# stelleg/caster-dta

Measured on AMD Instinct MI355X. Metric: graph-pairs/sec (Davis-shaped protein+drug), encoders fwd+bwd, higher is better.
Workload: dtype f32; 1 GPU; davis_b64; pairs_per_gpu=64, residues_per_gpu=19200, protein_edges_per_gpu=57484, atoms_per_gpu=2560, drug_edges_per_gpu=7986, encoder=CASTER-DTA(2,2), pass=fwdbwd, activation_storage=fp32, scope=encoders, torch_compile=False, tunable_gemms=False, two_lane_head=False, train_mode=True, csr_build_in_step=True, hip_graph=True, kernels=mfma

## Files before the change

caster-dta_amd/csrc/gvp_internal.h:

```cpp
#pragma once
#include <hip/hip_runtime.h>
#include <stdint.h>

#include "gvp_host.h"
#include "gvp_math.h"
#include "gvp_rng.h"

constexpr int POLICY_F32 = 0, POLICY_BF16 = 1, POLICY_GVPDEF = 2, POLICY_LINEAR = 3;

struct QuadOffsets {
  int emb, conv0, node0, layer_stride, head, total;
  int embT, convT0, nodeT0, layerT_stride, headT;
};

#ifndef CGVP_BWD_MAX_GRID
#define CGVP_BWD_MAX_GRID 240
#endif
constexpr int kBwdMaxGrid = CGVP_BWD_MAX_GRID;

#include <type_traits>

namespace gq { struct bf16s; struct f32_gvpdef; struct f32_linear; }
template <class T> struct Tag { using type = T; };
template <class ST> constexpr bool is_layer_kind = std::is_same_v<ST, gq::f32_gvpdef> || std::is_same_v<ST, gq::f32_linear>;
// ... 10 lines not shown
template <class F>
int with_flag(bool b, F&& f) { return b ? f(std::true_type{}) : f(std::false_type{}); }

namespace quad {
int offsets(int nt_node, int nt_edge, int num_convs, QuadOffsets* o);
int prepare(const gvp::EncLayout& L, int num_convs, int packed_bf16, const float* params, float* image, hipStream_t st);
int node_embed(int nt_node, const float* img, const float* x_s, const float* x_v, const int64_t* ntypes,
               int64_t N, float* h, unsigned long long* rng_state, unsigned long long* rng_out, int policy, hipStream_t st);
int pass_begin(const gvp::EncLayout& L, int num_convs, int policy, const float* params, float* image, const float* x_s,
               const float* x_v, const int64_t* ntypes, int64_t N, float* h, unsigned long long* rng_state,
               unsigned long long* rng_out, const int64_t* edge_index, int64_t E, int32_t* counters, hipStream_t st);
int conv(int nt_edge, const float* img, const float* h, const float* e_s, const float* e_v,
         const int64_t* etypes, const int32_t* rowptr, const int32_t* eperm, const int32_t* esrc,
         const int32_t* edst, int64_t N, int64_t E, int mean, float* dh, int fuse, const float* img_node,
         const float* img_head, float* h_out, float* out, const float* mask0, const float* mask1, gvp::RngArgs rng,
         const float* e_in, float* e_out, int policy, hipStream_t st);
int node_update(const float* img_node, const float* img_head, const float* h, const float* dh, int64_t N,
                int with_head, float* h_out, float* out, const float* mask0, const float* mask1, gvp::RngArgs rng,
                int policy, hipStream_t st);

int node_update_bwd(const float* img_node, const float* imgT_node, const float* h, const float* dh,
                    const float* mask0, const float* mask1, gvp::RngArgs rng, const float* g_up0, const float* g_up1,
                    const float* g_up2, int64_t N, float* g_dh, float* g_h, float* zero_rows, float* slab, int* grid,
                    int policy, hipStream_t st);
int head_bwd(const float* img_head, const float* imgT_head, const float* h_out, const float* g_out, int64_t N,
             float* g_h_out, float* slab, int* grid, int policy, hipStream_t st);
int node_head_bwd(const float* img_head, const float* imgT_head, const float* h_out, const float* g_out, float* g_h_out,
                  float* head_slab, const float* img_node, const float* imgT_node, const float* h, const float* dh,
                  const float* mask0, const float* mask1, gvp::RngArgs rng, int64_t N, float* g_dh, float* g_h,
                  float* zero_rows, float* slab, int* grid, int policy, hipStream_t st);
int conv_bwd(int nt_edge, const float* img, const float* imgT, const float* h, const float* e_emb,
// ... 29 lines not shown
             int* row_len, hipStream_t st, const float* agg_in = nullptr, const uint16_t* pos_in = nullptr,
             float* g_edge = nullptr, float* g_self = nullptr,
             float* g_eattr = nullptr, int eattr_accum = 0);
int gine_fwd(int cin, int chid, int cout, int nt, int net, int ed, const float* x, const int64_t* ntypes,
             const float* eattr, const int64_t* etypes, const int32_t* rowptr, const int32_t* eperm,
             const int32_t* esrc, const int32_t* edst, int64_t N, const cgvp_gine_w* w, float slope,
             const float* mask, gvp::RngArgs rng, float* out, float* agg_out, uint16_t* pos_out, hipStream_t st);
int reduce_slab(const float* slab, int rows, int stride, int col0, int len, float* dst, hipStream_t st);
int reduce_segments(const cgvp_segment* segs, int nsegs, float* grad_params, hipStream_t st, int overwrite = 0,
                    bool store_only = false);
struct BwdBlocks { int emb, conv_edge, conv_total, node, head; };
int bwd_block_sizes(int nt_node, int nt_edge, BwdBlocks* b);
void zero_words(void* p, size_t words, hipStream_t s);
int csr_build(const int64_t* edge_index, int64_t N, int64_t E, int32_t* rowptr, int32_t* eperm, int32_t* esrc,
              int32_t* edst, int32_t* work, int work_is_zero, int32_t* ids_scratch, unsigned long long* rng_state,
              unsigned long long* rng_out, hipStream_t stream);
}
```

caster-dta_amd/csrc/gvp_kernels.hip:

```cpp
#include <hip/hip_runtime.h>
#include <stdlib.h>
#include <stdint.h>

#include "gvp_internal.h"

using namespace gvp;

namespace {

constexpr int WAVE = 64;

inline int check_dims(const cgvp_dims* d) {
  if (!d) return CGVP_ERR_BAD_ARG;
  if (d->node_in_s != NODE_IN_S || d->node_in_v != NODE_IN_V || d->edge_in_s != EDGE_IN_S ||
      d->edge_in_v != EDGE_IN_V || d->hidden_s != NS || d->hidden_v != NV ||
      d->edge_hidden_s != ES || d->edge_hidden_v != EV || d->out_s != OUT)
    return CGVP_ERR_UNSUPPORTED_DIMS;
  if (d->storage != CGVP_F32 && d->storage != CGVP_BF16) return CGVP_ERR_UNSUPPORTED_DIMS;
  if (d->layer_kind < CGVP_LAYER_GATED || d->layer_kind > CGVP_LAYER_LINEAR) return CGVP_ERR_UNSUPPORTED_DIMS;
  if (d->layer_kind != CGVP_LAYER_GATED && d->storage != CGVP_F32) return CGVP_ERR_UNSUPPORTED_DIMS;
  return 0;
}
inline int check_dims_gated(const cgvp_dims* d) {
  if (int rc = check_dims(d)) return rc;
// ... 41 lines not shown
  int64_t e = (int64_t)blockIdx.x * blockDim.x + threadIdx.x;
  if (rng_state && e == 0) {
    const unsigned long long off = rng_state[1] + 1;
    rng_state[1] = off;
    rng_out[0] = rng_state[0];
    rng_out[1] = off;
  }
  if (e >= E) return;
  int64_t s = ei[e], d = ei[E + e];
  if (s < 0 || s >= N || d < 0 || d >= N) return;
  atomicAdd(&cnt[d], 1);
}

constexpr int SCAN_LDS = 36 * 1024;
__global__ __launch_bounds__(1024) void csr_scan_kernel(const int32_t* __restrict__ cnt, int64_t N,
                                                        int32_t* __restrict__ rowptr) {
  extern __shared__ int32_t sbuf[];
  const int t = threadIdx.x;
  const int tile_cap = (int)(N < SCAN_LDS ? (N + 3) / 4 * 4 : SCAN_LDS);
  int32_t* part = sbuf + tile_cap;
  int32_t carry = 0;
  for (int64_t base = 0; base < N || base == 0; base += SCAN_LDS) {
    const int64_t rem = N - base;
    const int n = (int)(rem < SCAN_LDS ? (rem > 0 ? rem : 0) : SCAN_LDS);
    constexpr int VPT = SCAN_LDS / 4096;
    int4 v[VPT];
    const int n4 = n >> 2;
    const int4* src4 = reinterpret_cast<const int4*>(cnt + base);
#pragma unroll
    for (int k = 0; k < VPT; ++k) {
      const int q = t + 1024 * k;
      v[k] = q < n4 ? src4[q] : make_int4(0, 0, 0, 0);
    }
// ... 37 lines not shown
        reinterpret_cast<int4*>(rowptr + base)[q] = x;
      }
      if (t < (n & 3)) rowptr[base + (n4 << 2) + t] = sbuf[(n4 << 2) + t];
    } else {
      for (int i = t; i < n; i += 1024) rowptr[base + i] = sbuf[i];
    }
    carry += total;
    __syncthreads();
    if (N == 0) break;
  }
  if (t == 0) rowptr[N] = carry;
}

constexpr int SCAN_MULTI_MAX = 65536, SCAN_MULTI_T = 256, SCAN_MULTI_CHUNK = 4 * SCAN_MULTI_T;
__global__ __launch_bounds__(SCAN_MULTI_T) void csr_scan_multi_kernel(const int32_t* __restrict__ cnt, int32_t N,
                                                                      int32_t counters, int32_t* __restrict__ rowptr) {
  __shared__ int32_t part[2 * (SCAN_MULTI_T / WAVE)];
  const int t = threadIdx.x, wv = t >> 6;
  const int4* c4 = reinterpret_cast<const int4*>(cnt);
  int32_t pre = 0;
  for (int q = t; q < (int)blockIdx.x * SCAN_MULTI_T; q += SCAN_MULTI_T) {
    const int4 v = c4[q];
    pre += (v.x + v.y) + (v.z + v.w);
  }
  const int i0 = (int)blockIdx.x * SCAN_MULTI_CHUNK + 4 * t;
  const int4 v = i0 < counters ? c4[i0 >> 2] : make_int4(0, 0, 0, 0);
  const int32_t sum = (v.x + v.y) + (v.z + v.w);
  int32_t inc = sum;
#pragma unroll
  for (int off = 1; off < WAVE; off <<= 1) {
    const int32_t u = __shfl_up(inc, off);
    if ((t & (WAVE - 1)) >= off) inc += u;
    pre += __shfl_xor(pre, off);
// ... 14 lines not shown
  }
}

__global__ void csr_fill_kernel(const int64_t* __restrict__ ei, int64_t N, int64_t E, const int32_t* __restrict__ rowptr,
                                int32_t* __restrict__ cnt, int32_t* __restrict__ tmp, int32_t* __restrict__ edst) {
  int64_t e = (int64_t)blockIdx.x * blockDim.x + threadIdx.x;
  if (e >= E) return;
  int64_t s = ei[e], d = ei[E + e];
  if (s < 0 || s >= N || d < 0 || d >= N) return;
  int32_t pos = rowptr[d] + atomicSub(&cnt[d], 1) - 1;
  if (pos < 0 || pos >= E) return;
  tmp[pos] = (int32_t)e;
  edst[pos] = (int32_t)d;
}

__global__ void csr_rank_kernel(const int64_t* __restrict__ ei, int64_t N, int64_t E, int64_t counters,
                                const int32_t* __restrict__ rowptr, const int32_t* __restrict__ tmp,
                                int32_t* __restrict__ edst, int32_t* __restrict__ eperm,
                                int32_t* __restrict__ esrc, int32_t* __restrict__ cnt) {
  const int64_t t = (int64_t)blockIdx.x * blockDim.x + threadIdx.x;
  if (t < counters) cnt[t] = 0;
  if (t >= rowptr[N] || t >= E) {
    if (t < E) { eperm[t] = -1; esrc[t] = 0; edst[t] = 0; }
    return;
  }
  const int32_t n = edst[t];
  if (n < 0 || n >= N) return;
  int32_t lo = rowptr[n], hi = rowptr[n + 1];
  const int32_t key = tmp[t];
  if (lo < 0 || hi > E || lo > hi || key < 0 || key >= E) return;
  int32_t rank = 0;
  for (int32_t j = lo; j < hi; ++j) rank += tmp[j] < key ? 1 : 0;
  eperm[lo + rank] = key;
  esrc[lo + rank] = (int32_t)ei[key];
}

__global__ void src_count_kernel(const int32_t* __restrict__ esrc, const int32_t* __restrict__ rowptr, int64_t N,
                                 int32_t* __restrict__ cnt) {
  const int64_t p = (int64_t)blockIdx.x * blockDim.x + threadIdx.x;
  if (p >= rowptr[N]) return;
  const int32_t s = esrc[p];
  if (s >= 0 && s < N) atomicAdd(&cnt[s], 1);
}
__global__ void src_fill_kernel(const int32_t* __restrict__ esrc, const int32_t* __restrict__ rowptr, int64_t N,
                                const int32_t* __restrict__ sptr, int32_t* __restrict__ cnt, int32_t* __restrict__ tmp) {
  const int64_t p = (int64_t)blockIdx.x * blockDim.x + threadIdx.x;
  const int32_t ev = rowptr[N];
  if (p >= ev) return;
  const int32_t s = esrc[p];
// ... 396 lines not shown
const char* cgvp_build_info(void) { return "libcaster_gvp gfx950 (HIP, wave64), built " __DATE__ " " __TIME__; }

int cgvp_csr_from_coo(const int64_t* edge_index, int64_t N, int64_t E, int32_t* rowptr,
                      int32_t* eperm, int32_t* esrc, int32_t* edst, int32_t* work, int32_t work_is_zero,
                      int32_t* ids_scratch, void* stream) {
  return quad::csr_build(edge_index, N, E, rowptr, eperm, esrc, edst, work, work_is_zero, ids_scratch, nullptr, nullptr,
                         (hipStream_t)stream);
}
}

namespace quad {
void zero_words(void* p, size_t words, hipStream_t s) { ::zero_words(p, words, s); }

int csr_build(const int64_t* edge_index, int64_t N, int64_t E, int32_t* rowptr, int32_t* eperm, int32_t* esrc,
              int32_t* edst, int32_t* work, int work_is_zero, int32_t* ids_scratch, unsigned long long* rng_state,
              unsigned long long* rng_out, hipStream_t stream) {
  if (N < 0 || E < 0 || !rowptr || !work || (E > 0 && (!edge_index || !eperm || !esrc || !edst || !ids_scratch)))
    return CGVP_ERR_BAD_ARG;
  if (N >= (int64_t)1 << 31 || E >= (int64_t)1 << 31) return CGVP_ERR_BAD_ARG;
  if ((uintptr_t)work & 15) return CGVP_ERR_BAD_ARG;
  hipStream_t s = stream;
  const int64_t counters = (N + 1 + 63) / 64 * 64;
  if (work_is_zero == 0) {
    zero_words(work, (size_t)counters, s);
  }
  int32_t* tmp = ids_scratch;
  const int B = 256;
  if (E > 0 && work_is_zero != 2)
    launch<csr_count_kernel>(dim3((unsigned)((E + B - 1) / B)), dim3(B), 0, s, edge_index, N, E, work, rng_state, rng_out);
  else if (rng_state)
    launch<rng_next_kernel>(dim3(1), dim3(1), 0, s, rng_state, rng_out);
  if (N < SCAN_MULTI_MAX) {
    launch<csr_scan_multi_kernel>(dim3((unsigned)((N + 1 + SCAN_MULTI_CHUNK - 1) / SCAN_MULTI_CHUNK)),
                                  dim3(SCAN_MULTI_T), 0, s, work, (int32_t)N, (int32_t)counters, rowptr);
  } else {
    const int64_t tile = N < SCAN_LDS ? (N + 3) / 4 * 4 : SCAN_LDS;
    if (int rc = launch<csr_scan_kernel>(dim3(1), dim3(1024), (size_t)(tile + 1024 + 32) * sizeof(int32_t), s, work, N, rowptr)) return rc;
  }
  if (E > 0) launch<csr_fill_kernel>(dim3((unsigned)((E + B - 1) / B)), dim3(B), 0, s, edge_index, N, E, rowptr, work, tmp, edst);
  const int64_t span = E > counters ? E : counters;
  launch<csr_rank_kernel>(dim3((unsigned)((span + B - 1) / B)), dim3(B), 0, s, edge_index, N, E, counters, rowptr, tmp,
                          edst, eperm, esrc, work);
  return launch_status();
}

bool deterministic_env() {
  static const bool v = [] { const char* e = getenv("CGVP_DETERMINISTIC"); return e && e[0] == '1'; }();
  return v;
}

int64_t src_index_work_ints(int64_t N, int64_t E) { return (N + 1 + 63) / 64 * 64 + (E > 0 ? E : 1); }

int src_index(const int32_t* rowptr, const int32_t* esrc, int64_t N, int64_t E, int32_t* sptr, int32_t* spos,
              int32_t* work, hipStream_t s) {
  if (N < 0 || E < 0 || !rowptr || !sptr || !work || (E > 0 && (!esrc || !spos))) return CGVP_ERR_BAD_ARG;
  if (N >= (int64_t)1 << 31 || E >= (int64_t)1 << 31 || ((uintptr_t)work & 15)) return CGVP_ERR_BAD_ARG;
  const int64_t counters = (N + 1 + 63) / 64 * 64;
  int32_t* cnt = work;
  int32_t* tmp = work + counters;
  zero_words(cnt, (size_t)counters, s);
  const int B = 256;
  const unsigned eb = (unsigned)((E + B - 1) / B);
  if (E > 0) launch<src_count_kernel>(dim3(eb), dim3(B), 0, s, esrc, rowptr, N, cnt);
  if (N < SCAN_MULTI_MAX) {
    launch<csr_scan_multi_kernel>(dim3((unsigned)((N + 1 + SCAN_MULTI_CHUNK - 1) / SCAN_MULTI_CHUNK)),
                                  dim3(SCAN_MULTI_T), 0, s, cnt, (int32_t)N, (int32_t)counters, sptr);
  } else {
    const int64_t tile = N < SCAN_LDS ? (N + 3) / 4 * 4 : SCAN_LDS;
    if (int rc = launch<csr_scan_kernel>(dim3(1), dim3(1024), (size_t)(tile + 1024 + 32) * sizeof(int32_t), s, cnt, N, sptr)) return rc;
  }
  if (E > 0) {
    launch<src_fill_kernel>(dim3(eb), dim3(B), 0, s, esrc, rowptr, N, sptr, cnt, tmp);
    launch<src_rank_kernel>(dim3(eb), dim3(B), 0, s, esrc, rowptr, N, sptr, tmp, spos);
  }
  return launch_status();
}
}

extern "C" {

int cgvp_deterministic_forced(void) { return quad::deterministic_env() ? 1 : 0; }

int cgvp_csr_collate(const int32_t* st_rowptr, const int32_t* st_eperm, const int32_t* st_esrc,
                     const int32_t* st_edst, const int64_t* st_node_off, const int64_t* st_edge_off,
// ... 121 lines not shown
  hipStream_t st = (hipStream_t)stream;
  switch (layout->nt_edge) {
    case 0: launch<conv_fwd_kernel<0>>(grid, dim3(WAVE), 0, st, a); break;
    case 1: launch<conv_fwd_kernel<1>>(grid, dim3(WAVE), 0, st, a); break;
    default: return CGVP_ERR_UNSUPPORTED_DIMS;
  }
  return launch_status();
}

int cgvp_conv_layer_fwd(const cgvp_dims* dims, const cgvp_layout* layout, const float* image, int32_t layer,
                        const float* h, const float* e_s, const float* e_v, const int64_t* etypes,
                        const int32_t* rowptr, const int32_t* eperm, const int32_t* esrc, const int32_t* edst,
                        int64_t N, int64_t E, int32_t aggr_mean, const float* mask0, const float* mask1,
                        const cgvp_rng* rng, int32_t with_head, const float* e_in, float* e_out, float* dh,
                        float* h_out, float* out, void* stream) {
  if (int rc = check_dims_gated(dims)) return rc;
  if (int rc = check_rng(rng)) return rc;
  if (N < 0 || E < 0 || !layout || !image) return CGVP_ERR_BAD_ARG;
  if (layer < 0 || layer >= num_convs_of(*layout)) return CGVP_ERR_BAD_ARG;
  if (N == 0) return 0;
  if (!h || !rowptr || (with_head ? !out : !h_out)) return CGVP_ERR_BAD_ARG;
  if (E > 0 && (!esrc || !edst)) return CGVP_ERR_BAD_ARG;
  if (E > 0 && !e_in && (!e_s || !e_v || !eperm || (layout->nt_edge > 0 && !etypes))) return CGVP_ERR_BAD_ARG;
  const void* al[] = {h, e_s, dh, h_out, out, mask0, mask1, e_in, e_out};
  for (const void* q : al) if ((uintptr_t)q & 15) return CGVP_ERR_BAD_ARG;
  QuadOffsets o;
  if (int rc = quad::offsets(layout->nt_node, layout->nt_edge, num_convs_of(*layout), &o)) return rc;
  if (int rc = quad::conv(layout->nt_edge, image + o.conv0 + layer * o.layer_stride, h, e_s, e_v, etypes, rowptr, eperm,
                          esrc, edst, N, E, aggr_mean ? 1 : 0, dh, with_head ? 2 : 1,
                          image + o.node0 + layer * o.layer_stride, image + o.head, h_out, out, mask0, mask1,
                          rng_args(rng, 2 * layer), e_in, e_in ? nullptr : e_out, policy_of(dims), (hipStream_t)stream)) return rc;
  return launch_status();
}

int cgvp_node_update_fwd(const cgvp_dims* dims, const cgvp_layout* layout, const float* params,
                         const float* image, int32_t layer, const float* h, const float* dh, int64_t N,
                         int32_t with_head, float* h_out, float* out, void* stream) {
  if (int rc = check_dims(dims)) return rc;
  if (N < 0 || !layout || !params) return CGVP_ERR_BAD_ARG;
  if (layer < 0 || layer >= num_convs_of(*layout)) return CGVP_ERR_BAD_ARG;
  if (N == 0) return 0;
  if (!h || !dh || (with_head ? !out : !h_out)) return CGVP_ERR_BAD_ARG;
  if (((uintptr_t)h & 15) || ((uintptr_t)dh & 15)) return CGVP_ERR_BAD_ARG;
  if (image) {
    if (((uintptr_t)h_out & 15) || ((uintptr_t)out & 15)) return CGVP_ERR_BAD_ARG;
    QuadOffsets o;
    if (int rc = quad::offsets(layout->nt_node, layout->nt_edge, num_convs_of(*layout), &o)) return rc;
    if (int rc = quad::node_update(image + o.node0 + layer * o.layer_stride, image + o.head, h, dh, N,
// ... 291 lines not shown
```

caster-dta_amd/csrc/gvp_quad_kernels.hip:

```cpp
#include <hip/hip_runtime.h>
#include <stdlib.h>
#include <stdint.h>

#include "gvp_internal.h"
#include "gvp_quad.h"

using namespace gq;

namespace {

#ifdef CGVP_STAMPS
__device__ unsigned long long* g_stamp_buf = nullptr;
#define STAMP(slot)                                                                          \
  do {                                                                                       \
    __builtin_amdgcn_sched_barrier(0);                                                       \
    unsigned long long t_;                                                                   \
    asm volatile("s_waitcnt vmcnt(0) lgkmcnt(0)\n\ts_memtime %0\n\ts_waitcnt lgkmcnt(0)" : "=s"(t_)::"memory"); \
    __builtin_amdgcn_sched_barrier(0);                                                       \
    if (g_stamp_buf && (threadIdx.x & 63) == 0)                                              \
      g_stamp_buf[((size_t)blockIdx.x * WPB + (threadIdx.x >> 6)) * 16 + (slot)] = t_;        \
  } while (0)
#define STAMP_REAL(slot)                                                                     \
  do {                                                                                       \
    unsigned long long t_;                                                                   \
// ... 20 lines not shown
  f4* d = reinterpret_cast<f4*>(lds);
  f4 v[IT];
#pragma unroll
  for (int k = 0; k < IT; ++k) {
    const int idx = tid + k * TPB;
    if (idx < NF4) v[k] = s[idx];
  }
#pragma unroll
  for (int k = 0; k < IT; ++k) {
    const int idx = tid + k * TPB;
    if (idx < NF4) d[idx] = v[k];
  }
}

template <int N0, int N1, int N2, int TPB = gq_fwd_tpb>
__device__ __forceinline__ void stage_slices(float* lds, const float* __restrict__ s0, const float* __restrict__ s1,
                                             const float* __restrict__ s2, int tid) {
  static_assert(N0 % 4 == 0 && N1 % 4 == 0 && N2 % 4 == 0, "image slices are whole float4s");
  constexpr int F0 = N0 / 4, F1 = N1 / 4, F2 = N2 / 4;
  constexpr int I0 = (F0 + TPB - 1) / TPB, I1 = (F1 + TPB - 1) / TPB, I2 = (F2 + TPB - 1) / TPB;
  f4* d = reinterpret_cast<f4*>(lds);
  f4 v0[I0 > 0 ? I0 : 1], v1[I1 > 0 ? I1 : 1], v2[I2 > 0 ? I2 : 1];
#pragma unroll
  for (int k = 0; k < I0; ++k) { const int idx = tid + k * TPB; if (idx < F0) v0[k] = reinterpret_cast<const f4*>(s0)[idx]; }
#pragma unroll
  for (int k = 0; k < I1; ++k) { const int idx = tid + k * TPB; if (idx < F1) v1[k] = reinterpret_cast<const f4*>(s1)[idx]; }
#pragma unroll
  for (int k = 0; k < I2; ++k) { const int idx = tid + k * TPB; if (idx < F2) v2[k] = reinterpret_cast<const f4*>(s2)[idx]; }
#pragma unroll
  for (int k = 0; k < I0; ++k) { const int idx = tid + k * TPB; if (idx < F0) d[idx] = v0[k]; }
#pragma unroll
  for (int k = 0; k < I1; ++k) { const int idx = tid + k * TPB; if (idx < F1) d[F0 + idx] = v1[k]; }
#pragma unroll
  for (int k = 0; k < I2; ++k) { const int idx = tid + k * TPB; if (idx < F2) d[F0 + F1 + idx] = v2[k]; }
}

template <int NTN, int NTE>
__device__ __forceinline__ float image_element(const float* __restrict__ P, const EncLayout& L, int num_convs, int packed, int idx) {
  typedef Image<NTN, NTE> IM;

  float v;
  if (idx < IM::EMB_SIZE) {
    v = idx < IM::EMB_LN ? QNode<NTN>::element(P + L.node_gvp, idx, packed != 0) : P[L.node_ln + (idx - IM::EMB_LN)];
  } else if (idx < IM::head(num_convs)) {
    const int j = idx - IM::EMB_SIZE;
    const int l = j / (IM::CV_SIZE + IM::ND_SIZE);
    int k = j - l * (IM::CV_SIZE + IM::ND_SIZE);
    const float* C = P + L.conv0 + l * L.conv_stride;
    if (k < IM::CV_SIZE) {
// ... 239 lines not shown
  f4 s[1], m1s;
  float v[3][1], m1v;
  node_inputs<ST, ST>(a, lane, active, n, a.dh, n * ROW, s, v, m1s, m1v);
  stage_slices<IM::ND_SIZE, (HEAD ? IM::HD_SIZE : 0), 0>(lds, a.img_node, a.img_head, nullptr, threadIdx.x);
  __syncthreads();
  node_tile<HEAD, ST>(lds, lds + IM::ND_SIZE, lane, active, n, s, v, m1s, m1v, a.h_out, a.out);
}

struct ConvQArgs {
  const float* img;
  const float* h; const float* e_s; const float* e_v; const int64_t* etypes;
  const int32_t* rowptr; const int32_t* eperm; const int32_t* esrc; const int32_t* edst;
  int64_t N; int npw; int mean; float* dh;
  NodeQArgs node;
  const float* e_in; float* e_out; int64_t E;
};
constexpr int EROW = 36;

constexpr int CTN = 2;

struct ConvIn {
  f4 es0[CTN], es1[CTN], sj[CTN], si[CTN];
  float ev[CTN][3], vj[CTN][3], vi[CTN][3];
  int et[CTN];
  int32_t dst[CTN];
  bool active[CTN];
};

template <int NTE, int EMODE, typename ST>
__device__ __forceinline__ void conv_gather(const ConvQArgs& a, int32_t base, int32_t e1, int lane, ConvIn& in) {
// ... 146 lines not shown

template <int NTE, int FUSE, int EMODE, typename ST, int CW = 4>
__global__ __launch_bounds__(WAVE * CW) __attribute__((amdgpu_waves_per_eu(2, 2))) void conv_quad_kernel(ConvQArgs a) {
  constexpr int WPB = CW, TPB = WAVE * CW;
  typedef Image<0, NTE> IM;
  typedef Image<0, 0> IMN;
  constexpr int ACC = WAVE * ROW;
  constexpr int ND_FLOATS = FUSE == 0 ? 0 : IMN::ND_SIZE + (FUSE == 2 ? IMN::HD_SIZE : 0);
  extern __shared__ __attribute__((aligned(16))) float lds[];
  float* img = lds;
  const int lane = threadIdx.x & 63, w = threadIdx.x >> 6;
  float* nd_img = lds + IM::CV_SIZE;
  float* acc = nd_img + ND_FLOATS + w * ACC;
  STAMP(0);
  STAMP_REAL(14);
  const int64_t n0 = ((int64_t)blockIdx.x * WPB + w) * a.npw;
  const int nn = n0 < a.N ? (int)((a.N - n0 < a.npw) ? (a.N - n0) : a.npw) : 0;
  const int32_t e0 = nn > 0 ? a.rowptr[n0] : 0, e1 = nn > 0 ? a.rowptr[n0 + nn] : 0;
  ConvIn in;
  conv_gather<NTE, EMODE, ST>(a, e0, e1, lane, in);
  if (EMODE == 1 && blockIdx.x == 0 && threadIdx.x < EROW / 4)
    Io<ST>::st4(a.e_out, a.E * EROW + 4 * threadIdx.x, f4{0.f, 0.f, 0.f, 0.f});
  stage_slices<IM::CV_SIZE, (FUSE > 0 ? IMN::ND_SIZE : 0), (FUSE == 2 ? IMN::HD_SIZE : 0), TPB>(
      img, a.img, a.node.img_node, a.node.img_head, threadIdx.x);
  for (int k = lane; k < nn * ROW; k += WAVE) acc[k] = 0.f;
  STAMP(1);
  __syncthreads();
  STAMP(2);

  const int i = lane & 15, g = lane >> 4;
  for (int32_t base = e0; base < e1; base += CTN * TILE) {
    if (base != e0) conv_gather<NTE, EMODE, ST>(a, base, e1, lane, in);
    const int32_t (&dst)[CTN] = in.dst;
    const bool (&active)[CTN] = in.active;
    f4 m_s[CTN];
    float m_v[CTN][3];
    STAMP(3);
    conv_tiles<NTE, EMODE, ST>(img, in, lane, a.e_out, a.E, base, m_s, m_v);
    STAMP(6);
// ... 167 lines not shown
template <int NTE, int FUSE>
int conv_launch(const ConvQArgs& a, int64_t grid, int policy, hipStream_t st) {
  return with_policy<NTE == 0 && FUSE == 0>(policy, [&](auto tag) {
    using ST = typename decltype(tag)::type;
    if constexpr (is_layer_kind<ST>)
      return a.e_in ? conv_launch_e<NTE, FUSE, 2, ST>(a, grid, st) : CGVP_ERR_UNSUPPORTED_DIMS;
    else
      return conv_launch_s<NTE, FUSE, ST>(a, grid, st);
  });
}

int conv(int nt_edge, const float* img, const float* h, const float* e_s, const float* e_v,
         const int64_t* etypes, const int32_t* rowptr, const int32_t* eperm, const int32_t* esrc,
         const int32_t* edst, int64_t N, int64_t E, int mean, float* dh, int fuse, const float* img_node,
         const float* img_head, float* h_out, float* out, const float* mask0, const float* mask1, gvp::RngArgs rng,
         const float* e_in, float* e_out, int policy, hipStream_t st) {
  int64_t deg = N > 0 ? (E + N - 1) / N : 1;
  if (deg < 1) deg = 1;
  int npw = (int)((CTN * TILE - 2) / deg);
  npw = npw < 1 ? 1 : (npw > WAVE ? WAVE : npw);
  if (fuse == 0) {
    const int64_t max_waves = 4 * 2048;
    if ((N + npw - 1) / npw > max_waves) {
      int64_t m = (N + max_waves - 1) / max_waves;
      npw = (int)(m > WAVE ? WAVE : m);
    }
  }
  ConvQArgs a{img, h, e_s, e_v, etypes, rowptr, eperm, esrc, edst, N, npw, mean, dh,
              NodeQArgs{img_node, img_head, h, nullptr, N, h_out, out, mask0, mask1, rng}, e_in, e_out, E};
  const int64_t groups = (N + npw - 1) / npw;
  const int64_t grid = groups;
  if (nt_edge != 0 && nt_edge != 1) return CGVP_ERR_UNSUPPORTED_DIMS;
  if (fuse < 0 || fuse > 2) return CGVP_ERR_BAD_ARG;
  if (nt_edge == 0) {
    if (fuse == 0) return conv_launch<0, 0>(a, grid, policy, st);
    if (fuse == 1) return conv_launch<0, 1>(a, grid, policy, st);
    return conv_launch<0, 2>(a, grid, policy, st);
  }
  if (fuse == 0) return conv_launch<1, 0>(a, grid, policy, st);
  if (fuse == 1) return conv_launch<1, 1>(a, grid, policy, st);
  return conv_launch<1, 2>(a, grid, policy, st);
}

int node_update(const float* img_node, const float* img_head, const float* h, const float* dh, int64_t N,
                int with_head, float* h_out, float* out, const float* mask0, const float* mask1, gvp::RngArgs rng,
// ... 15 lines not shown
```

caster-dta_amd/csrc/pass_api.hip:

```cpp
#include <hip/hip_runtime.h>
#include <stdint.h>
#include <stdlib.h>

#include <atomic>
#include <mutex>
#include <vector>

#include "gvp_internal.h"

namespace {

struct TimedLaunch { hipEvent_t a, b; int kind; };
std::atomic<bool> g_timing{false};
std::mutex g_timed_mutex;
std::vector<TimedLaunch> g_timed;
struct Timed {
  hipStream_t st; bool on; TimedLaunch t;
  Timed(int kind, void* stream) : st((hipStream_t)stream), on(g_timing.load(std::memory_order_relaxed)) {
    if (!on) return;
    t.kind = kind;
    if (hipEventCreate(&t.a) != hipSuccess || hipEventCreate(&t.b) != hipSuccess) { on = false; return; }
    (void)hipEventRecord(t.a, st);
  }
  ~Timed() {
// ... 148 lines not shown
int cgvp_lba_fwd_workspace(const cgvp_dims* dims, const cgvp_layout* layout, int64_t N, int64_t E, int32_t save_state,
                           cgvp_lba_fwd_ws* out) {
  if (!dims || !layout || !out || N < 0 || E < 0) return CGVP_ERR_BAD_ARG;
  if (dims->layer_kind != CGVP_LAYER_GATED) return CGVP_ERR_UNSUPPORTED_DIMS;
  const int64_t img = cgvp_lba_image_floats(dims, layout);
  if (img < 0) return (int)img;
  const int nc = num_convs_of(*layout);
  Bump b;
  out->seed = b.take(16);
  out->image = b.take(img * 4);
  out->state_rows = save_state ? 2 * nc + 1 : 3;
  out->node_stride = N + (N & 1);
  out->state = b.take(out->state_rows * out->node_stride * ROW * esize(dims));
  out->e_emb = b.take((E + 1) * EROW * esize(dims) > E * 4 ? (E + 1) * EROW * esize(dims) : E * 4);
  out->ids_scratch = out->e_emb;
  out->rowptr = b.take((N + 1) * 4);
  out->eperm = b.take((E > 0 ? E : 1) * 4);
  out->esrc = b.take((E > 0 ? E : 1) * 4);
  out->edst = b.take((E > 0 ? E : 1) * 4);
  out->total = b.off;
  return 0;
}

int cgvp_lba_forward_plan(int64_t N, int64_t E, int32_t num_convs, int32_t prebuilt_csr, int32_t flags, int32_t* fused_layers) {
  if (N < 0 || E < 0 || num_convs < 1) return CGVP_ERR_BAD_ARG;
  const int fuse = !(flags & CGVP_PASS_UNFUSED) && E <= 4 * N;
  if (fused_layers) *fused_layers = fuse;
  int launches = 1 + (prebuilt_csr ? 0 : (E > 0 ? 3 : 2));
  if (N > 0) launches += num_convs * (fuse ? 1 : 2);
  return launches;
}

int cgvp_lba_forward_pass(const cgvp_dims* dims, const cgvp_layout* layout, const float* params,
                          const cgvp_lba_batch* batch, int32_t aggr_mean, float dropout_p, uint64_t* rng_state,
                          const float* masks, int32_t* csr_counters, void* workspace, int32_t save_state,
                          int32_t flags, float* out, void* stream) {
  if (!dims || !layout || !params || !batch || !workspace) return CGVP_ERR_BAD_ARG;
  if ((uintptr_t)workspace & 255) return CGVP_ERR_BAD_ARG;
  const int64_t N = batch->num_nodes, E = batch->num_edges;
  cgvp_lba_fwd_ws ws;
  if (int rc = cgvp_lba_fwd_workspace(dims, layout, N, E, save_state, &ws)) return rc;
  const int nc = num_convs_of(*layout);
  if (nc < 1) return CGVP_ERR_UNSUPPORTED_DIMS;
// ... 4 lines not shown
  const bool tables = has_tables(batch);
  if (tables && (E > 0 && (!batch->eperm || !batch->esrc || !batch->edst))) return CGVP_ERR_BAD_ARG;
  if (!tables && E > 0 && (!batch->edge_index || !csr_counters)) return CGVP_ERR_BAD_ARG;
  if (N > 0 && !out) return CGVP_ERR_BAD_ARG;
  const int es = esize(dims);
  float* image = at<float>(workspace, ws.image);
  uint64_t* seed = at<uint64_t>(workspace, ws.seed);
  char* state = at<char>(workspace, ws.state);
  const int64_t srow = ws.node_stride * ROW * es;
  auto row = [&](int64_t r) { return reinterpret_cast<float*>(state + r * srow); };
  float* e_emb = at<float>(workspace, ws.e_emb);
  int32_t* rowptr = tables ? const_cast<int32_t*>(batch->rowptr) : at<int32_t>(workspace, ws.rowptr);
  int32_t* eperm = tables ? const_cast<int32_t*>(batch->eperm) : at<int32_t>(workspace, ws.eperm);
  int32_t* esrc = tables ? const_cast<int32_t*>(batch->esrc) : at<int32_t>(workspace, ws.esrc);
  int32_t* edst = tables ? const_cast<int32_t*>(batch->edst) : at<int32_t>(workspace, ws.edst);
  const bool count_here = !tables && E > 0;
  if (int rc = cgvp_lba_pass_begin(dims, layout, params, image, batch->x_s, batch->x_v, batch->ntypes, N, row(0),
                                   draw ? rng_state : nullptr, draw ? seed : nullptr,
                                   count_here ? batch->edge_index : nullptr, E, count_here ? csr_counters : nullptr, stream))
    return rc;
  if (!tables) {
    if (!csr_counters) return CGVP_ERR_BAD_ARG;
    if (int rc = cgvp_csr_from_coo(batch->edge_index, N, E, rowptr, eperm, esrc, edst, csr_counters, count_here ? 2 : 1,
                                   at<int32_t>(workspace, ws.ids_scratch), stream))
      return rc;
  }
  if (N == 0) return 0;
  int32_t fuse_i = 0;
  (void)cgvp_lba_forward_plan(N, E, nc, tables ? 1 : 0, flags, &fuse_i);
  const bool fuse = fuse_i != 0;
  const int64_t mstride = N * MROW;
  for (int l = 0; l < nc; ++l) {
    const bool last = l == nc - 1;
    cgvp_rng rng{draw ? seed : nullptr, dropout_p, 2 * l};
    const cgvp_rng* rp = draw ? &rng : nullptr;
    const float* m0 = (drop && masks) ? masks + (int64_t)(2 * l) * mstride : nullptr;
    const float* m1 = (drop && masks) ? masks + (int64_t)(2 * l + 1) * mstride : nullptr;
    float *h, *dh, *h_out;
    if (save_state) { h = row(l); dh = row(nc + l); h_out = last ? row(2 * nc) : row(l + 1); }
    else { h = row(l & 1); dh = fuse ? nullptr : row(2); h_out = last ? nullptr : row((l + 1) & 1); }
    const float* e_in = l > 0 ? e_emb : nullptr;
    float* e_out = l == 0 ? e_emb : nullptr;
    if (fuse) {
      Timed timed(0, stream);
      if (int rc = cgvp_conv_layer_fwd(dims, layout, image, l, h, batch->e_s, batch->e_v, batch->etypes, rowptr, eperm, esrc,
                                       edst, N, E, aggr_mean, m0, m1, rp, last ? 1 : 0, e_in, e_out, dh, h_out, out, stream))
        return rc;
    } else {
      {
        Timed timed(0, stream);
        if (int rc = cgvp_conv_fwd(dims, layout, params, image, l, h, batch->e_s, batch->e_v, batch->etypes, rowptr, eperm,
                                   esrc, edst, N, E, aggr_mean, e_in, e_out, dh, stream))
          return rc;
      }
      if (!save_state && last) h_out = row((l + 1) & 1);
      if (int rc = cgvp_node_update_fwd_train(dims, layout, image, l, h, dh, m0, m1, rp, N, last ? 1 : 0, h_out, out, stream))
        return rc;
    }
  }
  return launch_status();
}
// ... 354 lines not shown
```

caster-dta_amd/gvp_hip/autograd_ops.py:

```python
from __future__ import annotations

import ctypes as C
import math
import os
from typing import List, Tuple

import torch
from torch import Tensor

from . import _lib, ops
from .ops import _act, _f32, _i64, _ptr, _stream

MROW = 20
_CFG_FIELDS = ("node_in_s", "node_in_v", "edge_in_s", "edge_in_v", "hidden_s", "hidden_v", "edge_hidden_s",
               "edge_hidden_v", "out_s")
CFG_NTN, CFG_NTE, CFG_NC, CFG_MEAN, CFG_LEN = 9, 10, 11, 12, 13


PINNED_MASKS = None


def draw_seed(device):
    return torch.randint(0, 1 << 62, (2,), dtype=torch.int64, device=device)

# ... 56 lines not shown
    for p in params:
        if p.untyped_storage().data_ptr() != st.data_ptr() or p.storage_offset() != o or not p.is_contiguous():
            return torch.cat([q.detach().reshape(-1) for q in params])
        o += p.numel()
    return torch.empty(0, dtype=p0.dtype, device=p0.device).set_(st, off, (o - off,), (1,))


def _up(v, a=256):
    return (v + a - 1) // a * a


def lba_fwd_ws_bytes(N, E, num_convs, image_floats, esize, save_state):
    rows = 2 * num_convs + 1 if save_state else 3
    e1 = E if E > 0 else 1
    return (_up(16) + _up(image_floats * 4) + _up(rows * (N + N % 2) * ops.ROW * esize) + _up((E + 1) * ops.EROW * esize)
            + _up((N + 1) * 4) + 3 * _up(e1 * 4))


def gine_fwd_ws_bytes(N, E, widths, save_state, saved_only=False):
    L = len(widths) - 1
    e1 = E if E > 0 else 1
    if save_state:
        hidden = sum(_up(N * widths[l + 1] * 4) for l in range(L - 1))
        hidden += sum(_up(N * ((widths[l] + 15) // 16 * 16) * 4) + _up(e1 * 8) for l in range(L))
    else:
        hidden = 2 * _up(N * max([1] + list(widths[1:L])) * 4)
    return _up(16) + hidden + _up((N + 1) * 4) + (3 if saved_only else 4) * _up(e1 * 4)


def _csr_ptrs(csr):
    if len(csr) == 0:
# ... 510 lines not shown
```

caster-dta_amd/gvp_hip/ops.py:

```python
from __future__ import annotations

import ctypes as C
import os
from dataclasses import dataclass

import torch

from . import _lib
from ._lib import Dims, GineW, Layout, Rng
from ._lib import _on_gpu, _ptr, _stream

CASTER_DIMS = dict(node_in_s=17, node_in_v=3, edge_in_s=32, edge_in_v=1, hidden_s=16, hidden_v=4,
                   edge_hidden_s=32, edge_hidden_v=1, out_s=64, storage=0, layer_kind=0)
LAYER_GATED, LAYER_GVPDEF, LAYER_LINEAR = 0, 1, 2
F32, BF16 = 0, 1
ROW = 28
EROW = 36


def _f32(t, name):
    return _act(t, name, torch.float32, accepted=(torch.float32,))


def _act(t, name, dtype, accepted=(torch.float32, torch.bfloat16)):
    _on_gpu(t, name)
    if t.dtype not in accepted:
        raise TypeError(f"{name}: expected {' or '.join(str(d)[len('torch.'):] for d in accepted)}, got {t.dtype}")
    if t.dtype != dtype:
        t = t.to(dtype)
    t = t.contiguous()
    if t.data_ptr() % 16:
        t = t.clone()
# ... 322 lines not shown
```

Baseline: 276,500 graph-pairs/sec.

## Partition fused conv forward by fixed edge windows via ownership table

Adds an ownership table built during CSR construction, inside the rank kernel as extra blocks, or by a separate kernel when the CSR is prebuilt. It maps fixed windows of 30 edges to node ranges, so each wave of the fused conv forward handles an edge-balanced slice rather than a fixed node count. A validity flag falls back to node-count partitioning when a window cannot be expressed cleanly. It also hoists the image slice global loads into registers before the edge gather, so their latency overlaps with it. The cost is extra workspace, window-bound computation, and possibly more launched waves.

Result: no change. 276,500 graph-pairs/sec (-0.0%).

```diff
diff --git a/caster-dta_amd/csrc/gvp_internal.h b/caster-dta_amd/csrc/gvp_internal.h
--- a/caster-dta_amd/csrc/gvp_internal.h
+++ b/caster-dta_amd/csrc/gvp_internal.h
@@ -48,7 +48,11 @@
          const int64_t* etypes, const int32_t* rowptr, const int32_t* eperm, const int32_t* esrc,
          const int32_t* edst, int64_t N, int64_t E, int mean, float* dh, int fuse, const float* img_node,
          const float* img_head, float* h_out, float* out, const float* mask0, const float* mask1, gvp::RngArgs rng,
-         const float* e_in, float* e_out, int policy, hipStream_t st);
+         const float* e_in, float* e_out, int policy, hipStream_t st, const int32_t* own = nullptr);
+constexpr int kOwnQ = 30;
+constexpr int64_t own_windows(int64_t E) { return E / kOwnQ + 1; }
+constexpr int64_t own_ints(int64_t E) { return 4 + 2 * (own_windows(E) + 1); }
+constexpr int64_t own_offset_ints(int64_t N) { return (N + 1 + 3) / 4 * 4; }
 int node_update(const float* img_node, const float* img_head, const float* h, const float* dh, int64_t N,
                 int with_head, float* h_out, float* out, const float* mask0, const float* mask1, gvp::RngArgs rng,
                 int policy, hipStream_t st);
@@ -108,5 +112,12 @@
 void zero_words(void* p, size_t words, hipStream_t s);
 int csr_build(const int64_t* edge_index, int64_t N, int64_t E, int32_t* rowptr, int32_t* eperm, int32_t* esrc,
               int32_t* edst, int32_t* work, int work_is_zero, int32_t* ids_scratch, unsigned long long* rng_state,
-              unsigned long long* rng_out, hipStream_t stream);
+              unsigned long long* rng_out, hipStream_t stream, int32_t* own = nullptr);
+int own_table(const int32_t* rowptr, const int32_t* edst, int64_t N, int64_t E, int32_t* own, hipStream_t st);
+int conv_layer_fwd(const cgvp_dims* dims, const cgvp_layout* layout, const float* image, int32_t layer,
+                   const float* h, const float* e_s, const float* e_v, const int64_t* etypes,
+                   const int32_t* rowptr, const int32_t* eperm, const int32_t* esrc, const int32_t* edst,
+                   int64_t N, int64_t E, int32_t aggr_mean, const float* mask0, const float* mask1,
+                   const cgvp_rng* rng, int32_t with_head, const float* e_in, float* e_out, float* dh,
+                   float* h_out, float* out, void* stream, const int32_t* own);
 }
diff --git a/caster-dta_amd/csrc/gvp_kernels.hip b/caster-dta_amd/csrc/gvp_kernels.hip
--- a/caster-dta_amd/csrc/gvp_kernels.hip
+++ b/caster-dta_amd/csrc/gvp_kernels.hip
@@ -79,9 +79,10 @@
 
 constexpr int SCAN_LDS = 36 * 1024;
 __global__ __launch_bounds__(1024) void csr_scan_kernel(const int32_t* __restrict__ cnt, int64_t N,
-                                                        int32_t* __restrict__ rowptr) {
+                                                        int32_t* __restrict__ rowptr, int32_t* __restrict__ own) {
   extern __shared__ int32_t sbuf[];
   const int t = threadIdx.x;
+  if (own && t == 0) own[0] = 1;
   const int tile_cap = (int)(N < SCAN_LDS ? (N + 3) / 4 * 4 : SCAN_LDS);
   int32_t* part = sbuf + tile_cap;
   int32_t carry = 0;
@@ -149,9 +150,11 @@
 
 constexpr int SCAN_MULTI_MAX = 65536, SCAN_MULTI_T = 256, SCAN_MULTI_CHUNK = 4 * SCAN_MULTI_T;
 __global__ __launch_bounds__(SCAN_MULTI_T) void csr_scan_multi_kernel(const int32_t* __restrict__ cnt, int32_t N,
-                                                                      int32_t counters, int32_t* __restrict__ rowptr) {
+                                                                      int32_t counters, int32_t* __restrict__ rowptr,
+                                                                      int32_t* __restrict__ own) {
   __shared__ int32_t part[2 * (SCAN_MULTI_T / WAVE)];
   const int t = threadIdx.x, wv = t >> 6;
+  if (own && blockIdx.x == 0 && t == 0) own[0] = 1;
   const int4* c4 = reinterpret_cast<const int4*>(cnt);
   int32_t pre = 0;
   for (int q = t; q < (int)blockIdx.x * SCAN_MULTI_T; q += SCAN_MULTI_T) {
@@ -196,10 +199,43 @@
   edst[pos] = (int32_t)d;
 }
 
+__device__ __forceinline__ bool own_entry(const int32_t* __restrict__ rowptr, const int32_t* __restrict__ edst,
+                                          int32_t N, int64_t E, int64_t w, int32_t* __restrict__ own) {
+  const int64_t p = w * quad::kOwnQ;
+  const int32_t ev = rowptr[N];
+  const int32_t at = E > 0 ? edst[p < E ? p : E - 1] : 0;
+  bool ok = ev >= 0 && ev <= E;
+  int32_t t0 = N, e0 = ok ? ev : 0;
+  if (ok && p <= ev) {
+    int32_t n = N;
+    bool exact = true;
+    if (p < ev) {
+      n = at;
+      if (n < 0 || n >= N) { ok = false; n = N; }
+      else if (rowptr[n] != (int32_t)p) { t0 = n + 1; e0 = rowptr[n + 1]; exact = false; }
+    }
+    if (ok && exact) {
+      for (int k = 0; k < WAVE && n > 0 && rowptr[n - 1] == (int32_t)p; ++k) --n;
+      if (n > 0 && rowptr[n - 1] == (int32_t)p) ok = false;
+      t0 = n; e0 = (int32_t)p;
+    }
+  }
+  if (ok && (int64_t)t0 + WAVE < N && rowptr[t0 + WAVE] < (w + 1) * quad::kOwnQ) ok = false;
+  own[4 + 2 * w] = t0;
+  own[4 + 2 * w + 1] = e0;
+  return ok;
+}
+
 __global__ void csr_rank_kernel(const int64_t* __restrict__ ei, int64_t N, int64_t E, int64_t counters,
                                 const int32_t* __restrict__ rowptr, const int32_t* __restrict__ tmp,
                                 int32_t* __restrict__ edst, int32_t* __restrict__ eperm,
-                                int32_t* __restrict__ esrc, int32_t* __restrict__ cnt) {
+                                int32_t* __restrict__ esrc, int32_t* __restrict__ cnt, int32_t* __restrict__ own,
+                                unsigned rank_blocks) {
+  if (blockIdx.x >= rank_blocks) {
+    const int64_t w = (int64_t)(blockIdx.x - rank_blocks) * blockDim.x + threadIdx.x;
+    if (w <= quad::own_windows(E) && !own_entry(rowptr, edst, (int32_t)N, E, w, own)) own[0] = 0;
+    return;
+  }
   const int64_t t = (int64_t)blockIdx.x * blockDim.x + threadIdx.x;
   if (t < counters) cnt[t] = 0;
   if (t >= rowptr[N] || t >= E) {
@@ -215,6 +251,14 @@
   for (int32_t j = lo; j < hi; ++j) rank += tmp[j] < key ? 1 : 0;
   eperm[lo + rank] = key;
   esrc[lo + rank] = (int32_t)ei[key];
+}
+
+__global__ __launch_bounds__(1024) void own_table_kernel(const int32_t* __restrict__ rowptr, const int32_t* __restrict__ edst,
+                                                         int64_t N, int64_t E, int32_t* __restrict__ own) {
+  bool ok = true;
+  for (int64_t w = threadIdx.x; w <= quad::own_windows(E); w += 1024) ok = own_entry(rowptr, edst, (int32_t)N, E, w, own) && ok;
+  const int all_ok = __syncthreads_and(ok ? 1 : 0);
+  if (threadIdx.x == 0) own[0] = all_ok ? 1 : 0;
 }
 
 __global__ void src_count_kernel(const int32_t* __restrict__ esrc, const int32_t* __restrict__ rowptr, int64_t N,
@@ -641,7 +685,7 @@
 
 int csr_build(const int64_t* edge_index, int64_t N, int64_t E, int32_t* rowptr, int32_t* eperm, int32_t* esrc,
               int32_t* edst, int32_t* work, int work_is_zero, int32_t* ids_scratch, unsigned long long* rng_state,
-              unsigned long long* rng_out, hipStream_t stream) {
+              unsigned long long* rng_out, hipStream_t stream, int32_t* own) {
   if (N < 0 || E < 0 || !rowptr || !work || (E > 0 && (!edge_index || !eperm || !esrc || !edst || !ids_scratch)))
     return CGVP_ERR_BAD_ARG;
   if (N >= (int64_t)1 << 31 || E >= (int64_t)1 << 31) return CGVP_ERR_BAD_ARG;
@@ -659,16 +703,23 @@
     launch<rng_next_kernel>(dim3(1), dim3(1), 0, s, rng_state, rng_out);
   if (N < SCAN_MULTI_MAX) {
     launch<csr_scan_multi_kernel>(dim3((unsigned)((N + 1 + SCAN_MULTI_CHUNK - 1) / SCAN_MULTI_CHUNK)),
-                                  dim3(SCAN_MULTI_T), 0, s, work, (int32_t)N, (int32_t)counters, rowptr);
+                                  dim3(SCAN_MULTI_T), 0, s, work, (int32_t)N, (int32_t)counters, rowptr, own);
   } else {
     const int64_t tile = N < SCAN_LDS ? (N + 3) / 4 * 4 : SCAN_LDS;
-    if (int rc = launch<csr_scan_kernel>(dim3(1), dim3(1024), (size_t)(tile + 1024 + 32) * sizeof(int32_t), s, work, N, rowptr)) return rc;
+    if (int rc = launch<csr_scan_kernel>(dim3(1), dim3(1024), (size_t)(tile + 1024 + 32) * sizeof(int32_t), s, work, N, rowptr, own)) return rc;
   }
   if (E > 0) launch<csr_fill_kernel>(dim3((unsigned)((E + B - 1) / B)), dim3(B), 0, s, edge_index, N, E, rowptr, work, tmp, edst);
   const int64_t span = E > counters ? E : counters;
-  launch<csr_rank_kernel>(dim3((unsigned)((span + B - 1) / B)), dim3(B), 0, s, edge_index, N, E, counters, rowptr, tmp,
-                          edst, eperm, esrc, work);
-  return launch_status();
+  const unsigned rank_blocks = (unsigned)((span + B - 1) / B), own_blocks = own ? (unsigned)((own_windows(E) + 1 + B - 1) / B) : 0u;
+  launch<csr_rank_kernel>(dim3(rank_blocks + own_blocks), dim3(B), 0, s, edge_index, N, E, counters, rowptr, tmp,
+                          edst, eperm, esrc, work, own, rank_blocks);
+  return launch_status();
+}
+
+int own_table(const int32_t* rowptr, const int32_t* edst, int64_t N, int64_t E, int32_t* own, hipStream_t s) {
+  if (N < 0 || E < 0 || !rowptr || !own || (E > 0 && !edst)) return CGVP_ERR_BAD_ARG;
+  if (N >= (int64_t)1 << 31 || E >= (int64_t)1 << 31) return CGVP_ERR_BAD_ARG;
+  return launch<own_table_kernel>(dim3(1), dim3(1024), 0, s, rowptr, edst, N, E, own);
 }
 
 bool deterministic_env() {
@@ -691,10 +742,10 @@
   if (E > 0) launch<src_count_kernel>(dim3(eb), dim3(B), 0, s, esrc, rowptr, N, cnt);
   if (N < SCAN_MULTI_MAX) {
     launch<csr_scan_multi_kernel>(dim3((unsigned)((N + 1 + SCAN_MULTI_CHUNK - 1) / SCAN_MULTI_CHUNK)),
-                                  dim3(SCAN_MULTI_T), 0, s, cnt, (int32_t)N, (int32_t)counters, sptr);
+                                  dim3(SCAN_MULTI_T), 0, s, cnt, (int32_t)N, (int32_t)counters, sptr, (int32_t*)nullptr);
   } else {
     const int64_t tile = N < SCAN_LDS ? (N + 3) / 4 * 4 : SCAN_LDS;
-    if (int rc = launch<csr_scan_kernel>(dim3(1), dim3(1024), (size_t)(tile + 1024 + 32) * sizeof(int32_t), s, cnt, N, sptr)) return rc;
+    if (int rc = launch<csr_scan_kernel>(dim3(1), dim3(1024), (size_t)(tile + 1024 + 32) * sizeof(int32_t), s, cnt, N, sptr, (int32_t*)nullptr)) return rc;
   }
   if (E > 0) {
     launch<src_fill_kernel>(dim3(eb), dim3(B), 0, s, esrc, rowptr, N, sptr, cnt, tmp);
@@ -846,6 +897,17 @@
                         int64_t N, int64_t E, int32_t aggr_mean, const float* mask0, const float* mask1,
                         const cgvp_rng* rng, int32_t with_head, const float* e_in, float* e_out, float* dh,
                         float* h_out, float* out, void* stream) {
+  return quad::conv_layer_fwd(dims, layout, image, layer, h, e_s, e_v, etypes, rowptr, eperm, esrc, edst, N, E, aggr_mean,
+                              mask0, mask1, rng, with_head, e_in, e_out, dh, h_out, out, stream, nullptr);
+}
+}
+
+int quad::conv_layer_fwd(const cgvp_dims* dims, const cgvp_layout* layout, const float* image, int32_t layer,
+                         const float* h, const float* e_s, const float* e_v, const int64_t* etypes,
+                         const int32_t* rowptr, const int32_t* eperm, const int32_t* esrc, const int32_t* edst,
+                         int64_t N, int64_t E, int32_t aggr_mean, const float* mask0, const float* mask1,
+                         const cgvp_rng* rng, int32_t with_head, const float* e_in, float* e_out, float* dh,
+                         float* h_out, float* out, void* stream, const int32_t* own) {
   if (int rc = check_dims_gated(dims)) return rc;
   if (int rc = check_rng(rng)) return rc;
   if (N < 0 || E < 0 || !layout || !image) return CGVP_ERR_BAD_ARG;
@@ -861,9 +923,11 @@
   if (int rc = quad::conv(layout->nt_edge, image + o.conv0 + layer * o.layer_stride, h, e_s, e_v, etypes, rowptr, eperm,
                           esrc, edst, N, E, aggr_mean ? 1 : 0, dh, with_head ? 2 : 1,
                           image + o.node0 + layer * o.layer_stride, image + o.head, h_out, out, mask0, mask1,
-                          rng_args(rng, 2 * layer), e_in, e_in ? nullptr : e_out, policy_of(dims), (hipStream_t)stream)) return rc;
-  return launch_status();
-}
+                          rng_args(rng, 2 * layer), e_in, e_in ? nullptr : e_out, policy_of(dims), (hipStream_t)stream, own)) return rc;
+  return launch_status();
+}
+
+extern "C" {
 
 int cgvp_node_update_fwd(const cgvp_dims* dims, const cgvp_layout* layout, const float* params,
                          const float* image, int32_t layer, const float* h, const float* dh, int64_t N,
diff --git a/caster-dta_amd/csrc/gvp_quad_kernels.hip b/caster-dta_amd/csrc/gvp_quad_kernels.hip
--- a/caster-dta_amd/csrc/gvp_quad_kernels.hip
+++ b/caster-dta_amd/csrc/gvp_quad_kernels.hip
@@ -58,25 +58,36 @@
 }
 
 template <int N0, int N1, int N2, int TPB = gq_fwd_tpb>
+struct SliceRegs {
+  static_assert(N0 % 4 == 0 && N1 % 4 == 0 && N2 % 4 == 0, "image slices are whole float4s");
+  static constexpr int F0 = N0 / 4, F1 = N1 / 4, F2 = N2 / 4;
+  static constexpr int I0 = (F0 + TPB - 1) / TPB, I1 = (F1 + TPB - 1) / TPB, I2 = (F2 + TPB - 1) / TPB;
+  f4 v0[I0 > 0 ? I0 : 1], v1[I1 > 0 ? I1 : 1], v2[I2 > 0 ? I2 : 1];
+  __device__ __forceinline__ void load(const float* __restrict__ s0, const float* __restrict__ s1,
+                                       const float* __restrict__ s2, int tid) {
+#pragma unroll
+    for (int k = 0; k < I0; ++k) { const int idx = tid + k * TPB; if (idx < F0) v0[k] = reinterpret_cast<const f4*>(s0)[idx]; }
+#pragma unroll
+    for (int k = 0; k < I1; ++k) { const int idx = tid + k * TPB; if (idx < F1) v1[k] = reinterpret_cast<const f4*>(s1)[idx]; }
+#pragma unroll
+    for (int k = 0; k < I2; ++k) { const int idx = tid + k * TPB; if (idx < F2) v2[k] = reinterpret_cast<const f4*>(s2)[idx]; }
+  }
+  __device__ __forceinline__ void store(float* lds, int tid) const {
+    f4* d = reinterpret_cast<f4*>(lds);
+#pragma unroll
+    for (int k = 0; k < I0; ++k) { const int idx = tid + k * TPB; if (idx < F0) d[idx] = v0[k]; }
+#pragma unroll
+    for (int k = 0; k < I1; ++k) { const int idx = tid + k * TPB; if (idx < F1) d[F0 + idx] = v1[k]; }
+#pragma unroll
+    for (int k = 0; k < I2; ++k) { const int idx = tid + k * TPB; if (idx < F2) d[F0 + F1 + idx] = v2[k]; }
+  }
+};
+template <int N0, int N1, int N2, int TPB = gq_fwd_tpb>
 __device__ __forceinline__ void stage_slices(float* lds, const float* __restrict__ s0, const float* __restrict__ s1,
                                              const float* __restrict__ s2, int tid) {
-  static_assert(N0 % 4 == 0 && N1 % 4 == 0 && N2 % 4 == 0, "image slices are whole float4s");
-  constexpr int F0 = N0 / 4, F1 = N1 / 4, F2 = N2 / 4;
-  constexpr int I0 = (F0 + TPB - 1) / TPB, I1 = (F1 + TPB - 1) / TPB, I2 = (F2 + TPB - 1) / TPB;
-  f4* d = reinterpret_cast<f4*>(lds);
-  f4 v0[I0 > 0 ? I0 : 1], v1[I1 > 0 ? I1 : 1], v2[I2 > 0 ? I2 : 1];
-#pragma unroll
-  for (int k = 0; k < I0; ++k) { const int idx = tid + k * TPB; if (idx < F0) v0[k] = reinterpret_cast<const f4*>(s0)[idx]; }
-#pragma unroll
-  for (int k = 0; k < I1; ++k) { const int idx = tid + k * TPB; if (idx < F1) v1[k] = reinterpret_cast<const f4*>(s1)[idx]; }
-#pragma unroll
-  for (int k = 0; k < I2; ++k) { const int idx = tid + k * TPB; if (idx < F2) v2[k] = reinterpret_cast<const f4*>(s2)[idx]; }
-#pragma unroll
-  for (int k = 0; k < I0; ++k) { const int idx = tid + k * TPB; if (idx < F0) d[idx] = v0[k]; }
-#pragma unroll
-  for (int k = 0; k < I1; ++k) { const int idx = tid + k * TPB; if (idx < F1) d[F0 + idx] = v1[k]; }
-#pragma unroll
-  for (int k = 0; k < I2; ++k) { const int idx = tid + k * TPB; if (idx < F2) d[F0 + F1 + idx] = v2[k]; }
+  SliceRegs<N0, N1, N2, TPB> r;
+  r.load(s0, s1, s2, tid);
+  r.store(lds, tid);
 }
 
 template <int NTN, int NTE>
@@ -346,6 +357,7 @@
   int64_t N; int npw; int mean; float* dh;
   NodeQArgs node;
   const float* e_in; float* e_out; int64_t E;
+  const int32_t* own; int nwin;
 };
 constexpr int EROW = 36;
 
@@ -522,15 +534,32 @@
   float* acc = nd_img + ND_FLOATS + w * ACC;
   STAMP(0);
   STAMP_REAL(14);
-  const int64_t n0 = ((int64_t)blockIdx.x * WPB + w) * a.npw;
-  const int nn = n0 < a.N ? (int)((a.N - n0 < a.npw) ? (a.N - n0) : a.npw) : 0;
-  const int32_t e0 = nn > 0 ? a.rowptr[n0] : 0, e1 = nn > 0 ? a.rowptr[n0 + nn] : 0;
+  const int64_t wv = (int64_t)blockIdx.x * WPB + w;
+  int32_t by_win = 0, o0[2] = {0, 0}, o1[2] = {0, 0};
+  if (a.own) {
+    by_win = a.own[0];
+    if (wv < a.nwin) {
+      const int2 lo = reinterpret_cast<const int2*>(a.own + 4)[wv], hi = reinterpret_cast<const int2*>(a.own + 4)[wv + 1];
+      o0[0] = lo.x; o0[1] = lo.y; o1[0] = hi.x; o1[1] = hi.y;
+    }
+  }
+  const int64_t l0 = wv * a.npw;
+  const int ln = l0 < a.N ? (int)((a.N - l0 < a.npw) ? (a.N - l0) : a.npw) : 0;
+  const int32_t le0 = ln > 0 ? a.rowptr[l0] : 0, le1 = ln > 0 ? a.rowptr[l0 + ln] : 0;
+  SliceRegs<IM::CV_SIZE, (FUSE > 0 ? IMN::ND_SIZE : 0), (FUSE == 2 ? IMN::HD_SIZE : 0), TPB> image_regs;
+  image_regs.load(a.img, a.node.img_node, a.node.img_head, threadIdx.x);
+  int64_t n0 = l0;
+  int nn = ln;
+  int32_t e0 = le0, e1 = le1;
+  if (by_win) {
+    n0 = o0[0]; nn = o1[0] - o0[0]; e0 = o0[1]; e1 = o1[1];
+    if (n0 < 0 || nn < 0 || nn > WAVE || n0 + nn > a.N) { nn = 0; e0 = e1 = 0; }
+  }
   ConvIn in;
   conv_gather<NTE, EMODE, ST>(a, e0, e1, lane, in);
   if (EMODE == 1 && blockIdx.x == 0 && threadIdx.x < EROW / 4)
     Io<ST>::st4(a.e_out, a.E * EROW + 4 * threadIdx.x, f4{0.f, 0.f, 0.f, 0.f});
-  stage_slices<IM::CV_SIZE, (FUSE > 0 ? IMN::ND_SIZE : 0), (FUSE == 2 ? IMN::HD_SIZE : 0), TPB>(
-      img, a.img, a.node.img_node, a.node.img_head, threadIdx.x);
+  image_regs.store(img, threadIdx.x);
   for (int k = lane; k < nn * ROW; k += WAVE) acc[k] = 0.f;
   STAMP(1);
   __syncthreads();
@@ -728,7 +757,7 @@
          const int64_t* etypes, const int32_t* rowptr, const int32_t* eperm, const int32_t* esrc,
          const int32_t* edst, int64_t N, int64_t E, int mean, float* dh, int fuse, const float* img_node,
          const float* img_head, float* h_out, float* out, const float* mask0, const float* mask1, gvp::RngArgs rng,
-         const float* e_in, float* e_out, int policy, hipStream_t st) {
+         const float* e_in, float* e_out, int policy, hipStream_t st, const int32_t* own) {
   int64_t deg = N > 0 ? (E + N - 1) / N : 1;
   if (deg < 1) deg = 1;
   int npw = (int)((CTN * TILE - 2) / deg);
@@ -741,8 +770,12 @@
     }
   }
   ConvQArgs a{img, h, e_s, e_v, etypes, rowptr, eperm, esrc, edst, N, npw, mean, dh,
-              NodeQArgs{img_node, img_head, h, nullptr, N, h_out, out, mask0, mask1, rng}, e_in, e_out, E};
-  const int64_t groups = (N + npw - 1) / npw;
+              NodeQArgs{img_node, img_head, h, nullptr, N, h_out, out, mask0, mask1, rng}, e_in, e_out, E, nullptr, 0};
+  int64_t groups = (N + npw - 1) / npw;
+  if (fuse > 0 && own && own_windows(E) < ((int64_t)1 << 30)) {
+    a.own = own; a.nwin = (int)own_windows(E);
+    groups = groups > a.nwin ? groups : a.nwin;
+  }
   const int64_t grid = groups;
   if (nt_edge != 0 && nt_edge != 1) return CGVP_ERR_UNSUPPORTED_DIMS;
   if (fuse < 0 || fuse > 2) return CGVP_ERR_BAD_ARG;
diff --git a/caster-dta_amd/csrc/pass_api.hip b/caster-dta_amd/csrc/pass_api.hip
--- a/caster-dta_amd/csrc/pass_api.hip
+++ b/caster-dta_amd/csrc/pass_api.hip
@@ -186,7 +186,7 @@
   out->state = b.take(out->state_rows * out->node_stride * ROW * esize(dims));
   out->e_emb = b.take((E + 1) * EROW * esize(dims) > E * 4 ? (E + 1) * EROW * esize(dims) : E * 4);
   out->ids_scratch = out->e_emb;
-  out->rowptr = b.take((N + 1) * 4);
+  out->rowptr = b.take((quad::own_offset_ints(N) + quad::own_ints(E)) * 4);
   out->eperm = b.take((E > 0 ? E : 1) * 4);
   out->esrc = b.take((E > 0 ? E : 1) * 4);
   out->edst = b.take((E > 0 ? E : 1) * 4);
@@ -199,6 +199,7 @@
   const int fuse = !(flags & CGVP_PASS_UNFUSED) && E <= 4 * N;
   if (fused_layers) *fused_layers = fuse;
   int launches = 1 + (prebuilt_csr ? 0 : (E > 0 ? 3 : 2));
+  if (prebuilt_csr && fuse && N > 0) launches += 1;
   if (N > 0) launches += num_convs * (fuse ? 1 : 2);
   return launches;
 }
@@ -233,6 +234,7 @@
   int32_t* eperm = tables ? const_cast<int32_t*>(batch->eperm) : at<int32_t>(workspace, ws.eperm);
   int32_t* esrc = tables ? const_cast<int32_t*>(batch->esrc) : at<int32_t>(workspace, ws.esrc);
   int32_t* edst = tables ? const_cast<int32_t*>(batch->edst) : at<int32_t>(workspace, ws.edst);
+  int32_t* own = at<int32_t>(workspace, ws.rowptr) + quad::own_offset_ints(N);
   const bool count_here = !tables && E > 0;
   if (int rc = cgvp_lba_pass_begin(dims, layout, params, image, batch->x_s, batch->x_v, batch->ntypes, N, row(0),
                                    draw ? rng_state : nullptr, draw ? seed : nullptr,
@@ -240,14 +242,16 @@
     return rc;
   if (!tables) {
     if (!csr_counters) return CGVP_ERR_BAD_ARG;
-    if (int rc = cgvp_csr_from_coo(batch->edge_index, N, E, rowptr, eperm, esrc, edst, csr_counters, count_here ? 2 : 1,
-                                   at<int32_t>(workspace, ws.ids_scratch), stream))
+    if (int rc = quad::csr_build(batch->edge_index, N, E, rowptr, eperm, esrc, edst, csr_counters, count_here ? 2 : 1,
+                                 at<int32_t>(workspace, ws.ids_scratch), nullptr, nullptr, (hipStream_t)stream, own))
       return rc;
   }
   if (N == 0) return 0;
   int32_t fuse_i = 0;
   (void)cgvp_lba_forward_plan(N, E, nc, tables ? 1 : 0, flags, &fuse_i);
   const bool fuse = fuse_i != 0;
+  if (tables && fuse)
+    if (int rc = quad::own_table(rowptr, edst, N, E, own, (hipStream_t)stream)) return rc;
   const int64_t mstride = N * MROW;
   for (int l = 0; l < nc; ++l) {
     const bool last = l == nc - 1;
@@ -262,8 +266,8 @@
     float* e_out = l == 0 ? e_emb : nullptr;
     if (fuse) {
       Timed timed(0, stream);
-      if (int rc = cgvp_conv_layer_fwd(dims, layout, image, l, h, batch->e_s, batch->e_v, batch->etypes, rowptr, eperm, esrc,
-                                       edst, N, E, aggr_mean, m0, m1, rp, last ? 1 : 0, e_in, e_out, dh, h_out, out, stream))
+      if (int rc = quad::conv_layer_fwd(dims, layout, image, l, h, batch->e_s, batch->e_v, batch->etypes, rowptr, eperm, esrc,
+                                        edst, N, E, aggr_mean, m0, m1, rp, last ? 1 : 0, e_in, e_out, dh, h_out, out, stream, own))
         return rc;
     } else {
       {
diff --git a/caster-dta_amd/gvp_hip/autograd_ops.py b/caster-dta_amd/gvp_hip/autograd_ops.py
--- a/caster-dta_amd/gvp_hip/autograd_ops.py
+++ b/caster-dta_amd/gvp_hip/autograd_ops.py
@@ -94,7 +94,7 @@
     rows = 2 * num_convs + 1 if save_state else 3
     e1 = E if E > 0 else 1
     return (_up(16) + _up(image_floats * 4) + _up(rows * (N + N % 2) * ops.ROW * esize) + _up((E + 1) * ops.EROW * esize)
-            + _up((N + 1) * 4) + 3 * _up(e1 * 4))
+            + _up(((N + 1 + 3) // 4 * 4 + 4 + 2 * (E // ops.CONV_OWN_Q + 2)) * 4) + 3 * _up(e1 * 4))
 
 
 def gine_fwd_ws_bytes(N, E, widths, save_state, saved_only=False):
diff --git a/caster-dta_amd/gvp_hip/ops.py b/caster-dta_amd/gvp_hip/ops.py
--- a/caster-dta_amd/gvp_hip/ops.py
+++ b/caster-dta_amd/gvp_hip/ops.py
@@ -16,6 +16,7 @@
 F32, BF16 = 0, 1
 ROW = 28
 EROW = 36
+CONV_OWN_Q = 30
 
 
 def _f32(t, name):
```
